# speechLabBcCuny/onssen

Hardware: AMD Instinct MI355X
Metric: real_time_factor (higher is better)
Workload: dtype f32 as split-bf16 (bf16x3 MFMA, fp32 accumulate)

## Files before the change

### include/onssen_hip.h

```cpp
#ifndef ONSSEN_HIP_H
#define ONSSEN_HIP_H

#include <stddef.h>
#include <stdint.h>

#ifdef __cplusplus
extern "C" {
#endif

#define ONSSEN_ABI_VERSION 14

#define ONSSEN_OK 0
#define ONSSEN_E_ARG (-1)
#define ONSSEN_E_WORKSPACE (-2)
#define ONSSEN_E_ALIGN (-3)
#define ONSSEN_WAV_TRUNCATED 1
#define ONSSEN_WAV_E_OPEN (-16)
#define ONSSEN_WAV_E_FORMAT (-17)
#define ONSSEN_WAV_E_UNSUPPORTED (-18)
#define ONSSEN_WAV_E_SOME_FAILED (-19)

#define ONSSEN_BLSTM_SPLIT_ROWS 1
#define ONSSEN_BLSTM_BF16X3 2
#define ONSSEN_BLSTM_XCD 4
// ... 73 lines not shown
                           int group, float eps, float* C, int R, int64_t c_s0, int64_t c_s1, float* C2, int64_t c2_s0,
                           int64_t c2_s1, int bf16_only, void* stream);
int onssen_linear_x3p_norms(const uint16_t* a_img, int M, int K, const uint16_t* w_img, const float* bias, int N, int group,
                            float eps, float* C, float* inv_norm, void* stream);

int onssen_linear_x3p_resid(const uint16_t* a_img, int M, int K, const uint16_t* w_img, const float* bias, int N, int group,
                            float eps, const float* resid, int resid_mod, float* C, int R, int64_t c_s0, int64_t c_s1,
                            int bf16_only, void* stream);

#define ONSSEN_BLSTM_WS_HEADER_BYTES 32768
size_t onssen_blstm_workspace_bytes(int B, int T, int in_dim, int H, int L, int ug);
int onssen_blstm_y_image(int B, int T, int in_dim, int H, int L, int ug, size_t* offset_bytes, int* KB);
int onssen_blstm_x_image(int B, int T, int in_dim, int H, int L, int ug, size_t* offset_bytes, int* KB);
int onssen_blstm_forward_f32(const float* x, int64_t xs_b, int64_t xs_t, int B, int T, int in_dim, int H, int L,
                             int ug, const float* const* wih_p_host, const float* const* whh_p_host,
                             const float* const* bias_p_host, float* y, void* ws, size_t ws_bytes, int flags,
                             void* stream);

size_t onssen_blstm_pipe2_workspace_bytes(int B, int T, int in_dim, int H, int ug);
int onssen_blstm_pipe2_y_image(int B, int T, int in_dim, int H, int ug, size_t* offset_bytes, int* KB);
int onssen_blstm_pipe2_forward_f32(const float* x, int64_t xs_b, int64_t xs_t, int B, int T, int in_dim, int H, int ug,
                                   const float* const* wih_p_host, const float* const* whh_p_host,
                                   const float* const* bias_p_host, void* ws, size_t ws_bytes, int flags, void* stream);
int onssen_blstm_pipe2_forward_ragged_f32(const float* x, int64_t xs_b, int64_t xs_t, int B, int T_cap, int T, const int32_t* frames,
                                          int T_prev, const int32_t* frames_prev, int in_dim, int H, int ug,
                                          const float* const* wih_p_host, const float* const* whh_p_host,
                                          const float* const* bias_p_host, void* ws, size_t ws_bytes, int flags, void* stream);

#define ONSSEN_LSTM_BWD_STEPS 0
#define ONSSEN_LSTM_BWD_XCD 1
int onssen_lstm_train_forward_f32(const float* x, int64_t x_stride_b, int64_t x_stride_t, int B, int T, int in_dim, int H,
                                  int ug, const uint16_t* wih_img, const uint16_t* whh_x3, const float* bias_p, float* y,
                                  float* gates, float* cs, void* ws, size_t ws_bytes, void* stream);
int onssen_lstm_train_backward_img_f32(int B, int T, int H, int ug, const uint16_t* whh_img, const float* dy, const float* gates,
                                       const float* cs, void* ws, size_t ws_bytes, float* db_rows, uint16_t* dp_img, void* stream);
int onssen_lstm_train_forward_form_f32(const float* x, int64_t x_stride_b, int64_t x_stride_t, int B, int T, int in_dim, int H,
                                       int ug, const void* wih, const void* whh, const float* bias_p, float* y, float* gates,
                                       float* cs, void* ws, size_t ws_bytes, int flags, void* stream);
int64_t onssen_lstm_whhT_elems(int H, int ug);
int onssen_lstm_pack_whhT_bf16x3(const float* w_hh, int H, int ug, uint16_t* out, void* stream);
int64_t onssen_lstm_whhR_elems(int H, int ug);
int onssen_lstm_pack_whhR_bf16x3(const float* w_hh, int H, int ug, uint16_t* out, void* stream);
size_t onssen_lstm_train_backward_workspace_bytes(int B, int H, int ug, int form);
int onssen_lstm_train_backward_f32(int B, int T, int H, int ug, const uint16_t* whh_img, const float* dy, float* gates_dp,
                                   const float* cs, void* ws, size_t ws_bytes, int form, float* db_rows, void* stream);
int onssen_dropout_f32(const float* x, int64_t n, float p, uint64_t seed, float* out, void* stream);
// ... 215 lines not shown
```

### onssen_amd/_abi.py

```python
import ctypes as C
import os

EPI_BIAS, EPI_L2NORM, EPI_SIGMOID, EPI_RELU = 0, 1, 2, 3
ENHANCE_MSA, ENHANCE_PSA = 0, 1
EPI_BF16 = 0x100
ABI_VERSION = 14
WAV_TRUNCATED = 1
BLSTM_SPLIT_ROWS = 1
BLSTM_BF16X3 = 2
BLSTM_XCD = 4
BLSTM_FUSE_IN0 = 16
BLSTM_FUSE_TAIL = 32
BLSTM_BF16 = 64
BLSTM_G_READY = 128
BLSTM_WS_DIRTY = 65536
LSTM_BWD_STEPS, LSTM_BWD_XCD = 0, 1
DC_CLUSTER_LAUNCH_PER_ITERATION = 1
BLSTM_WS_HEADER = 32768
TASNET_GLN, TASNET_CLN, TASNET_BN = 0, 1, 2
TASNET_RELU, TASNET_SIGMOID, TASNET_SOFTMAX = 0, 1, 2
TASNET_RAGGED_MAX = 64
TASNET_F32, TASNET_BF16X3, TASNET_BF16 = 0, 1, 2

_vp, _i, _i64, _f, _sz = C.c_void_p, C.c_int, C.c_int64, C.c_float, C.c_size_t
# ... 7 lines not shown
    "onssen_lstm_geometry_x3": (_i, [_i, _i, C.POINTER(_i), C.POINTER(_i), C.POINTER(_i64)]),
    "onssen_lstm_pack_whh_bf16x3": (_i, [_vp, _i, _i, _vp, _vp]),
    "onssen_lstm_pack_wih_bf16x3": (_i, [_vp, _i, _i, _i, _vp, _vp]),
    "onssen_lstm_pack_f32": (_i, [_vp, _vp, _vp, _vp, _i, _i, _i, _i, _vp, _vp, _vp, _vp]),
    "onssen_lstm_pack_train_f32": (_i, [_i, _i, _i, _i, _vp, _vp, _vp, _vp, _vp, _vp, _vp, _vp, _vp, _vp]),
    "onssen_lstm_pack_wih_image_f32": (_i, [_vp, _vp, _vp, _i, _i, _i, _i, _vp, _vp, _vp, _vp]),
    "onssen_clip_adam_workspace_bytes": (_sz, [_vp, _i]),
    "onssen_clip_adam_f32": (_i, [_i, _vp, _vp, _vp, _vp, _vp, _f, C.c_double, C.c_double, C.c_double, C.c_double, _i, _i, _vp, _sz, _vp]),
    "onssen_head_pack_f32": (_i, [_vp, _vp, _i, _i, _i, _vp, _vp, _vp, _vp, _f, _vp, _vp, _vp]),
    "onssen_linear_f32": (_i, [_vp, _i64, _i64, _i, _i, _i, _vp, _i, _vp, _i, _i, _i, _f, _vp, _vp, _i64, _i64, _vp]),
    "onssen_linear_pack_bf16x3": (_i, [_vp, _i, _i, _i, _i, _vp, _vp]),
    "onssen_linear_bf16x3": (_i, [_vp, _i64, _i64, _i, _i, _i, _vp, _i, _vp, _i, _i, _i, _f, _vp, _vp, _i64, _i64, _vp]),
    "onssen_x3_image_f32": (_i, [_vp, _i64, _i64, _i, _i, _i, _vp, _vp]),
    "onssen_linear_x3p": (_i, [_vp, _i, _i, _vp, _vp, _i, _i, _i, _f, _vp, _i, _i64, _i64, _vp]),
    "onssen_linear_x3p_resid": (_i, [_vp, _i, _i, _vp, _vp, _i, _i, _f, _vp, _i, _vp, _i, _i64, _i64, _i, _vp]),
    "onssen_linear_x3p_pair": (_i, [_vp, _i, _i, _vp, _vp, _i, _i, _i, _f, _vp, _i, _i64, _i64, _vp, _i64, _i64, _i, _vp]),
    "onssen_blstm_workspace_bytes": (_sz, [_i, _i, _i, _i, _i, _i]),
    "onssen_blstm_y_image": (_i, [_i, _i, _i, _i, _i, _i, _vp, _vp]),
    "onssen_blstm_x_image": (_i, [_i, _i, _i, _i, _i, _i, _vp, _vp]),
    "onssen_blstm_forward_f32": (_i, [_vp, _i64, _i64, _i, _i, _i, _i, _i, _i, _pp, _pp, _pp, _vp, _vp, _sz, _i, _vp]),
    "onssen_blstm_pipe2_workspace_bytes": (_sz, [_i, _i, _i, _i, _i]),
    "onssen_blstm_pipe2_y_image": (_i, [_i, _i, _i, _i, _i, _vp, _vp]),
    "onssen_blstm_pipe2_forward_f32": (_i, [_vp, _i64, _i64, _i, _i, _i, _i, _i, _pp, _pp, _pp, _vp, _sz, _i, _vp]),
    "onssen_blstm_pipe2_forward_ragged_f32": (_i, [_vp, _i64, _i64, _i, _i, _i, _vp, _i, _vp, _i, _i, _i, _pp, _pp, _pp, _vp, _sz, _i, _vp]),
    "onssen_linear_x3p_batched": (_i, [_vp, _i64, _i, _i, _vp, _i64, _vp, _i, _vp, _i64, _i64, _i, _vp]),
    "onssen_linear_x3p_batched_split": (_i, [_vp, _i64, _i, _i, _vp, _i64, _vp, _i, _i, _vp, _i64, _i64, _i64, _i, _vp, _i64, _i64, _i64,
                                             _i, _vp]),
    "onssen_linear_x3p_batched_split_alt": (_i, [_vp, _i64, _i, _i, _vp, _i64, _vp, _i, _i, _vp, _i64, _i64, _i64, _i, _vp, _i64, _i64,
                                                 _i64, _i, _i, _vp]),
    "onssen_linear_x3t": (_i, [_vp, _vp, _i, _i, _i, _vp, _vp, _i64, _vp]),
    "onssen_lstm_wgrad_images_f32": (_i, [_vp, _vp, _vp, _i, _i, _i, _i, _i, _vp, _i, _vp, _i64, _i64, _i64, _vp, _i64, _i64, _i64, _vp]),
    "onssen_x3_image_t_f32": (_i, [_vp, _i64, _i, _i, _i, _vp, _vp]),
    "onssen_x3_image_both_f32": (_i, [_vp, _i64, _i, _i, _vp, _vp, _vp]),
    "onssen_x3_image_both_colsum_f32": (_i, [_vp, _i64, _i, _i, _vp, _vp, _vp, _vp]),
    "onssen_lstm_train_forward_f32": (_i, [_vp, _i64, _i64, _i, _i, _i, _i, _i, _vp, _vp, _vp, _vp, _vp, _vp, _vp, _sz, _vp]),
    "onssen_lstm_train_forward_form_f32": (_i, [_vp, _i64, _i64, _i, _i, _i, _i, _i, _vp, _vp, _vp, _vp, _vp, _vp, _vp, _sz, _i, _vp]),
    "onssen_lstm_whhT_elems": (_i64, [_i, _i]),
    "onssen_lstm_pack_whhT_bf16x3": (_i, [_vp, _i, _i, _vp, _vp]),
    "onssen_lstm_whhR_elems": (_i64, [_i, _i]),
    "onssen_lstm_pack_whhR_bf16x3": (_i, [_vp, _i, _i, _vp, _vp]),
    "onssen_lstm_train_backward_workspace_bytes": (_sz, [_i, _i, _i, _i]),
    "onssen_lstm_train_backward_f32": (_i, [_i, _i, _i, _i, _vp, _vp, _vp, _vp, _vp, _sz, _i, _vp, _vp]),
    "onssen_lstm_train_backward_img_f32": (_i, [_i, _i, _i, _i, _vp, _vp, _vp, _vp, _vp, _sz, _vp, _vp, _vp]),
    "onssen_dropout_f32": (_i, [_vp, _i64, _f, C.c_uint64, _vp, _vp]),
    "onssen_l2norm_rows_f32": (_i, [_vp, _i64, _i, _f, _vp, _vp]),
    "onssen_bn_rows_workspace_bytes": (_sz, [_i64, _i]),
# ... 382 lines not shown
        if frames is not None:
            self.check(self.dll.onssen_blstm_forward_ragged_f32(x, xs_b, xs_t, B, T, frames, in_dim, H, L, ug, arr(*wih_ptrs),
                                                                arr(*whh_ptrs), arr(*bias_ptrs), y, ws, ws_bytes, flags, stream),
                       "onssen_blstm_forward_ragged_f32")
            return
        self.check(self.dll.onssen_blstm_forward_f32(x, xs_b, xs_t, B, T, in_dim, H, L, ug, arr(*wih_ptrs),
                                                     arr(*whh_ptrs), arr(*bias_ptrs), y, ws, ws_bytes, flags, stream),
                   "onssen_blstm_forward_f32")

    def blstm_pipe2_workspace_bytes(self, B, T, in_dim, H, ug):
        return int(self.dll.onssen_blstm_pipe2_workspace_bytes(B, T, in_dim, H, ug))

    def blstm_pipe2_y_image(self, B, T, in_dim, H, ug):
        off, kb = C.c_size_t(0), C.c_int(0)
        self.check(self.dll.onssen_blstm_pipe2_y_image(B, T, in_dim, H, ug, C.byref(off), C.byref(kb)), "onssen_blstm_pipe2_y_image")
        return int(off.value), int(kb.value)

    def blstm_pipe2_forward(self, x, xs_b, xs_t, B, T, in_dim, H, ug, wih_ptrs, whh_ptrs, bias_ptrs, ws, ws_bytes, flags, stream):
        arr = C.c_void_p * 2
        self.check(self.dll.onssen_blstm_pipe2_forward_f32(x, xs_b, xs_t, B, T, in_dim, H, ug, arr(*wih_ptrs), arr(*whh_ptrs),
                                                           arr(*bias_ptrs), ws, ws_bytes, flags, stream),
                   "onssen_blstm_pipe2_forward_f32")

    def blstm_pipe2_forward_ragged(self, x, xs_b, xs_t, B, T_cap, T, frames, T_prev, frames_prev, in_dim, H, ug, wih_ptrs, whh_ptrs,
                                   bias_ptrs, ws, ws_bytes, flags, stream):
        arr = C.c_void_p * 2
        self.check(self.dll.onssen_blstm_pipe2_forward_ragged_f32(x, xs_b, xs_t, B, T_cap, T, frames, T_prev, frames_prev, in_dim, H, ug,
                                                                  arr(*wih_ptrs), arr(*whh_ptrs), arr(*bias_ptrs), ws, ws_bytes, flags,
                                                                  stream),
                   "onssen_blstm_pipe2_forward_ragged_f32")

    def linear_x3p_batched(self, a_img, a_bs, M, K, w_img, w_bs, bias, N, out, c_bs, ldc, batch, stream):
        self.check(self.dll.onssen_linear_x3p_batched(a_img, a_bs, M, K, w_img, w_bs, bias, N, out, c_bs, ldc, batch, stream),
                   "onssen_linear_x3p_batched")

    def linear_x3p_batched_split(self, a_img, a_bs, M, K, w_img, w_bs, bias, N, R, out, c_bs, c_s0, c_s1, n_split, out2, c2_bs,
                                 c2_s0, c2_s1, batch, stream):
        self.check(self.dll.onssen_linear_x3p_batched_split(a_img, a_bs, M, K, w_img, w_bs, bias, N, R, out, c_bs, c_s0, c_s1, n_split,
                                                            out2, c2_bs, c2_s0, c2_s1, batch, stream), "onssen_linear_x3p_batched_split")

    def linear_x3p_batched_split_alt(self, a_img, a_bs, M, K, w_img, w_bs, bias, N, R, out, c_bs, c_s0, c_s1, n_split, out2, c2_bs,
                                     c2_s0, c2_s1, n_split_odd, batch, stream):
        self.check(self.dll.onssen_linear_x3p_batched_split_alt(a_img, a_bs, M, K, w_img, w_bs, bias, N, R, out, c_bs, c_s0, c_s1,
                                                                n_split, out2, c2_bs, c2_s0, c2_s1, n_split_odd, batch, stream),
                   "onssen_linear_x3p_batched_split_alt")

# ... 213 lines not shown
```

### onssen_amd/csrc/labels_cluster.inc

```
__global__ void utt_max_kernel(const float* __restrict__ x, long per_utt, float* __restrict__ out) {
  __shared__ float red[256];
  const float* p = x + (long)blockIdx.x * per_utt;
  float m = -INFINITY;
  for (long i = threadIdx.x; i < per_utt; i += 256) m = fmaxf(m, p[i]);
  red[threadIdx.x] = m;
  __syncthreads();
  for (int s = 128; s > 0; s >>= 1) {
    if ((int)threadIdx.x < s) red[threadIdx.x] = fmaxf(red[threadIdx.x], red[threadIdx.x + s]);
    __syncthreads();
  }
  if (threadIdx.x == 0) out[blockIdx.x] = red[0];
}

__global__ void labels_kernel(const float* __restrict__ mix, const float* __restrict__ s1, const float* __restrict__ s2,
                              const float* __restrict__ feat, const float* __restrict__ fmax, long per_utt, long total,
                              float db_threshold, float* __restrict__ one_hot, float* __restrict__ mag_mix,
                              float* __restrict__ mag_s1, float* __restrict__ mag_s2, float* __restrict__ cos_s1,
                              float* __restrict__ cos_s2) {
  for (long e = (long)blockIdx.x * blockDim.x + threadIdx.x; e < total; e += (long)gridDim.x * blockDim.x) {
    const float xr = mix[2 * e], xi = mix[2 * e + 1];
    const float ar = s1[2 * e], ai = s1[2 * e + 1], br = s2[2 * e], bi = s2[2 * e + 1];
    const float m1 = hypotf(ar, ai), m2 = hypotf(br, bi);
    mag_mix[e] = hypotf(xr, xi);
    mag_s1[e] = m1;
// ... 760 lines not shown
  for (long t0 = i_lo; t0 < i_hi; t0 += 256) {
    const long i = t0 + tid;
    const int act = (i < i_hi && f[i] >= thr) ? 1 : 0;
    scan[tid] = act;
    __syncthreads();
    for (int off = 1; off < 256; off <<= 1) {
      const int v = tid >= off ? scan[tid - off] : 0;
      __syncthreads();
      scan[tid] += v;
      __syncthreads();
    }
    if (i < i_hi) dst[i] = act ? base + scan[tid] - act : -1;
    const int tot = scan[255];
    __syncthreads();
    base += tot;
  }
  for (long i = nb + (long)blockIdx.x * 256 + tid; i < per_utt; i += (long)NBLK * 256) dst[i] = -1;
  if (blockIdx.x == 0) {
    float* wb = const_cast<float*>(ws) + (long)b * ws_stride;
    for (int k = tid; k < 2 * NBP * (D + 4); k += 256) wb[1 + 2 * D + k] = __builtin_bit_cast(float, 1u);
  }
}

template <int DT>
__global__ __launch_bounds__(256) void kmeans2_mask_compact_kernel(const float* __restrict__ comp, const int* __restrict__ dest,
                                                                   long per_utt, int D_rt, const float* __restrict__ ws,
                                                                   long ws_stride, float* __restrict__ masks) {
  using namespace km;
  constexpr int DC = DT ? DT : DMAX;
  const int D = DT ? DT : D_rt;
  const int b = blockIdx.y, tid = threadIdx.x;
  const float* e = comp + (long)b * per_utt * D;
  const int* dst = dest + (long)b * per_utt;
  const float* w = ws + (long)b * ws_stride;
  float c0[DC], c1[DC];
  float q0 = 0.f, q1 = 0.f;
#pragma unroll
  for (int d = 0; d < DC; ++d) {
    c0[d] = d < D ? w[1 + d] : 0.f; c1[d] = d < D ? w[1 + D + d] : 0.f;
    q0 += c0[d] * c0[d]; q1 += c1[d] * c1[d];
  }
  for (long i = (long)blockIdx.x * 256 + tid; i < per_utt; i += (long)gridDim.x * 256) {
    const int row = dst[i];
    int lab = 0;
    if (row >= 0) {
      float v[DC];
// ... 24 lines not shown
```

### onssen_amd/csrc/lstm.inc

```
struct StepArgs {
  const float* G = nullptr;
  const float* whh = nullptr;
  float* y = nullptr;
  float* c = nullptr;
  const unsigned short* whh_x3 = nullptr;
  unsigned short* hs = nullptr;
  int KQ2 = 0, Hs = 0;
  int B = 0, T = 0, Hp = 0, NP = 0, KQ = 0, NU = 0, step = 0;
  long long* dbg = nullptr;
  int ablate = 0;
  const int* frames = nullptr;
  float* save_g = nullptr;
  float* save_c = nullptr;
};

namespace rec {
constexpr int RLD = 72;
constexpr int QB = 10;
constexpr int QB3 = 5;
}

__device__ __forceinline__ float gate_sigmoid(float x) {
  return __builtin_amdgcn_rcpf(1.0f + __builtin_amdgcn_exp2f(-1.4426950408889634f * x));
}
// ... 296 lines not shown
  const unsigned short* ximg = nullptr;
  const float* bias0 = nullptr;
  int KC0 = 0;
  int KCM = 0;
  const float* x0 = nullptr;
  long xs_b = 0, xs_t = 0;
  const float* wtail = nullptr;
  float* save_g = nullptr;
  float* save_c = nullptr;
  int terms = 0;
  int RG = 0;
  unsigned spin_limit = 0;
  long long* dbg = nullptr;
  int ablate = 0;
  unsigned short* yimg = nullptr;
  int KBI = 0;
  const int* frames = nullptr;
  int nbg_a = 0;
  const float* G_b = nullptr;
  const unsigned short* whh_b = nullptr;
  unsigned short* yimg_b = nullptr;
  int T_b = 0;
  const int* frames_b = nullptr;
};

template <int J>
__device__ __forceinline__ unsigned quad_bcast(unsigned v) {
  return (unsigned)__builtin_amdgcn_update_dpp(0, (int)v, J * 0x55, 0xf, 0xf, false);
}

template <int NT, int NW, bool FUSE, int TERMS, bool STACK, bool SAVE = false, bool RAGGED = false>
__global__ __launch_bounds__(64 * NW) void lstm_xcd_kernel(XcdArgs p) {
  static_assert(!STACK || TERMS == 3, "stacking is a property of the split form");
  constexpr bool F32 = TERMS == 0;
  static_assert(!F32 || (!FUSE && !SAVE), "the exact-fp32 form is the plain inference recurrence");
  static_assert(NW == 8, "waves 5..7 never own elements: they stage the input projection");
  static_assert(!RAGGED || (TERMS == 3 && STACK && !FUSE && !SAVE), "ragged batches: the plain stacked split-bf16 inference recurrence");
  constexpr int UG = 4 * NT;
  constexpr int NE = 16 * UG;
  constexpr int NTHR = 64 * NW;
  constexpr int EPT = (NE + NTHR - 1) / NTHR;
  constexpr bool PAIRED = ONSSEN_XCD_PAIRED && STACK && !FUSE && NT >= 2;
  constexpr int NTA = PAIRED ? (NT + 1) / 2 : NT;
  constexpr int NKP = PAIRED ? 4 : NW;
  constexpr int CPW = F32 ? 40 / NW + (40 % NW != 0) : PAIRED ? 5 : 20 / NW + (20 % NW != 0);
  constexpr int CHB = F32 ? 1024 : 2048;
  constexpr int NHL = TERMS == 3 ? 2 : 1;
  constexpr int NLD = (TERMS == 3 && !STACK) ? 2 : 1;
  constexpr int PBS = 320, PTS = 4 * PBS + 16;
  constexpr unsigned TAG = F32 ? 0x40000000u : 0x4000u;
  constexpr int NGRP = tile_group_count(ONSSEN_XCD_TILE_GROUPS);
  constexpr bool GROUPED = !F32 && !PAIRED && NGRP > 1 && tile_group_sum(ONSSEN_XCD_TILE_GROUPS) == NT;
  __shared__ __attribute__((aligned(16))) char part_s[2 * NKP * NT * PTS];
  __shared__ __attribute__((aligned(16))) u32x4 share_s[PAIRED ? 4 * CPW * NLD * 64 : 1];
  __shared__ unsigned share_flag[4];
  constexpr int KCMAX = 4;
  __shared__ unsigned s_ctl[3];
  __shared__ unsigned s_done[8];
#ifndef ONSSEN_XCD_PROFILE_STN
#define ONSSEN_XCD_PROFILE_STN 64
#endif
  constexpr int ST0 = 64, STN = ONSSEN_XCD_PROFILE_STN;
  constexpr bool PROF = ONSSEN_XCD_PROFILE != 0;
  constexpr int ABL = ONSSEN_XCD_ABLATE;
  constexpr int DELAY_CELL = ONSSEN_XCD_DELAY_CELL ? ONSSEN_XCD_DELAY_CELL : (!STACK && TERMS == 3 && !FUSE) ? ONSSEN_XCD_DELAY_CELL_U
                             : (STACK && !SAVE) ? ONSSEN_XCD_DELAY_CELL_S : SAVE ? ONSSEN_XCD_DELAY_CELL_T : 0;
  constexpr int CELL_PRIO = ONSSEN_XCD_CELL_PRIO ? ONSSEN_XCD_CELL_PRIO : (!STACK && TERMS == 3 && !FUSE) ? ONSSEN_XCD_CELL_PRIO_U : 0;
  __shared__ long long stamp_s[PROF ? STN * 24 : 1];
  const int tid = threadIdx.x, lane = tid & 63;
  const int wave = __builtin_amdgcn_readfirstlane(tid >> 6);
  const int ugi = blockIdx.x >> 3, g = (p.ablate & 8) ? ((blockIdx.x + ugi) & 7) : (blockIdx.x & 7);
  if (PROF && p.dbg && tid == 0)
    p.dbg[4096 + blockIdx.x] = (long long)(__builtin_amdgcn_s_getreg(6164) & 15u) |
                               ((long long)__builtin_amdgcn_s_getreg(63492) << 8);
  if (g >= 2 * p.nbg) return;
  const int dir = g / p.nbg;
  int bg = g % p.nbg;
  if (p.nbg_a > 0 && bg >= p.nbg_a) {
    bg -= p.nbg_a;
    p.G = p.G_b; p.whh = p.whh_b; p.yimg = p.yimg_b; p.y = nullptr;
    if constexpr (RAGGED) { p.T = p.T_b; p.frames = p.frames_b; }
  }
  const int RG = p.RG;
  const int b0 = p.row0 + bg * RG;
  unsigned* abort_w = p.sync + 280;
  const long hx_group = (long)g * 2 * p.KQ2 * 1024;
  const int KQX = F32 ? (p.Hp + 15) / 16 : p.KQ2;

  const int qj = tid & 3;
  const unsigned lo_delta = STACK ? (unsigned)RG * 16u : 1024u;
  const long g_step = (long)p.B * 2 * p.NP, y_step = (long)p.B * 2 * p.Hp, i_step = (long)p.B * p.KBI * 64;
  bool e_ok[EPT], e_inb[EPT];
  unsigned g_off[EPT], y_off[EPT];
// ... 657 lines not shown
```

### onssen_amd/csrc/lstm_run.inc

```

struct LstmGeo {
  int ug, Hp, NP, NU;
  int KQ;
  int KQ2, Hs;
  int KQB, NUB;
};
static bool lstm_geo(int H, int ug, LstmGeo* g) {
  if (H <= 0 || ug < 4 || ug > 24 || (ug % 4) != 0) return false;
  g->ug = ug; g->Hp = ceil_div(H, ug) * ug; g->NP = 4 * g->Hp; g->NU = g->Hp / ug;
  g->KQ = ceil_div(g->Hp, 16); g->KQ2 = ceil_div(g->Hp, 32); g->Hs = 32 * g->KQ2;
  g->KQB = ceil_div(g->NP, 32); g->NUB = ceil_div(g->Hp, 16);
  return true;
}
int onssen_lstm_geometry(int H, int ug, int* Hp, int* NP, int* KQ, int64_t* whh_elems) {
  LstmGeo g;
  if (!lstm_geo(H, ug, &g)) return ONSSEN_E_ARG;
  if (Hp) *Hp = g.Hp;
  if (NP) *NP = g.NP;
  if (KQ) *KQ = g.KQ;
  if (whh_elems) *whh_elems = (int64_t)g.NU * g.KQ * (ug / 4) * 256;
  return ONSSEN_OK;
}
int onssen_lstm_geometry_x3(int H, int ug, int* KQ2, int* Hs, int64_t* whh_x3_elems) {
  LstmGeo g;
// ... 135 lines not shown
    } else if constexpr (NT < 6) {
      if (xa.terms == 0) {
        ONSSEN_XCD_LAUNCH(false, 0, false, false, false);
      } else if (xa.terms == 1) {
        if (fz) ONSSEN_XCD_LAUNCH(true, 1, false, false, false); else ONSSEN_XCD_LAUNCH(false, 1, false, false, false);
      } else {
        if (stack) ONSSEN_XCD_LAUNCH(true, 3, true, false, false); else ONSSEN_XCD_LAUNCH(true, 3, false, false, false);
      }
    }
  }
#undef ONSSEN_XCD_LAUNCH
  hipError_t e = hipGetLastError();
  return e == hipSuccess ? ONSSEN_OK : (int)e;
}

template <int NT>
static int launch_xcd_pair(XcdArgs xa, hipStream_t st) {
  if (xa.B > 32 || xa.terms != 3 || xa.KC0 > 0 || xa.save_c || !xa.G_b || !xa.whh_b || !xa.yimg_b) return ONSSEN_E_ARG;
  if ((xa.frames != nullptr) != (xa.frames_b != nullptr) || (xa.frames && xa.B > 16)) return ONSSEN_E_ARG;
  xa.RG = xa.B <= 16 ? 8 : 16;
  xa.row0 = 0;
  xa.nbg_a = ceil_div(xa.B, xa.RG);
  xa.nbg = 2 * xa.nbg_a;
  const dim3 grid((unsigned)(8 * xa.NU));
  if (xa.frames) hipLaunchKernelGGL((lstm_xcd_kernel<NT, 8, false, 3, true, false, true>), grid, dim3(512), 0, st, xa);
  else if (xa.RG == 8) hipLaunchKernelGGL((lstm_xcd_kernel<NT, 8, false, 3, true, false>), grid, dim3(512), 0, st, xa);
  else hipLaunchKernelGGL((lstm_xcd_kernel<NT, 8, false, 3, false, false>), grid, dim3(512), 0, st, xa);
  hipError_t e = hipGetLastError();
  return e == hipSuccess ? ONSSEN_OK : (int)e;
}

struct BlstmRun {
  const float* x; int64_t xs_b, xs_t; int B, T, in_dim, L, flags;
  const float* const* wih; const float* const* whh; const float* const* bias;
  float *y, *save_g, *save_c; const int32_t* frames; void* stream;
  LstmGeo g; BlstmWs o; char* ws;
  float *G, *ybuf; uint16_t *img_x, *img_ab[2]; long long* dbg;
  bool x3, xcd;
  bool images;
  bool bf16_only;
  bool fuse0(int l) const { return images && l == 0 && (flags & ONSSEN_BLSTM_FUSE_IN0); }
  float* yout(int l) const { return (L - 1 - l) % 2 == 0 ? y : ybuf; }
  const float* yin(int l) const { return (L - 1 - l) % 2 == 0 ? ybuf : y; }
};

static int blstm_plan(BlstmRun& r, int H, int ug, void* ws, size_t ws_bytes) {
  const int flags = r.flags;
  if (!lstm_geo(H, ug, &r.g)) return ONSSEN_E_ARG;
// ... 155 lines not shown
  return blstm_forward_impl(x, xs_b, xs_t, B, T, in_dim, H, L, ug, wih_p_host, whh_p_host, bias_p_host, y, ws, ws_bytes,
                            flags, stream, nullptr, nullptr, frames);
}

int onssen_lstm_train_forward_f32(const float* x, int64_t xs_b, int64_t xs_t, int B, int T, int in_dim, int H, int ug,
                                  const uint16_t* wih_img, const uint16_t* whh_x3, const float* bias_p, float* y,
                                  float* gates, float* cs, void* ws, size_t ws_bytes, void* stream) {
  return onssen_lstm_train_forward_form_f32(x, xs_b, xs_t, B, T, in_dim, H, ug, wih_img, whh_x3, bias_p, y, gates, cs, ws, ws_bytes,
                                            ONSSEN_BLSTM_BF16X3 | ONSSEN_BLSTM_XCD, stream);
}

int onssen_lstm_train_forward_form_f32(const float* x, int64_t xs_b, int64_t xs_t, int B, int T, int in_dim, int H, int ug,
                                       const void* wih, const void* whh, const float* bias_p, float* y, float* gates,
                                       float* cs, void* ws, size_t ws_bytes, int flags, void* stream) {
  if (!y || !gates || !cs || !aligned16(gates)) return ONSSEN_E_ARG;
  const int form = flags & (ONSSEN_BLSTM_XCD | ONSSEN_BLSTM_BF16X3);
  if ((flags & ~(ONSSEN_BLSTM_XCD | ONSSEN_BLSTM_BF16X3)) != 0 || form == ONSSEN_BLSTM_XCD) return ONSSEN_E_ARG;
  const float* wih_a[1] = {(const float*)wih};
  const float* whh_a[1] = {(const float*)whh};
  const float* bias[1] = {bias_p};
  return blstm_forward_impl(x, xs_b, xs_t, B, T, in_dim, H, 1, ug, wih_a, whh_a, bias, y, ws, ws_bytes, flags, stream, gates, cs);
}

static int blstm_pipe2_impl(const float* x, int64_t xs_b, int64_t xs_t, int B, int T_cap, int T, const int32_t* frames, int T_prev,
                            const int32_t* frames_prev, int in_dim, int H, int ug, const float* const* wih_p_host,
                            const float* const* whh_p_host, const float* const* bias_p_host, void* ws, size_t ws_bytes, int flags,
                            void* stream) {
  LstmGeo g;
  Pipe2Ws o;
  if (!lstm_geo(H, ug, &g)) return ONSSEN_E_ARG;
  if (!x || !ws || !wih_p_host || !whh_p_host || !bias_p_host || B <= 0 || B > 32 || T <= 0 || in_dim <= 0) return ONSSEN_E_ARG;
  if (T > T_cap || T_prev <= 0 || T_prev > T_cap) return ONSSEN_E_ARG;
  if ((frames != nullptr) != (frames_prev != nullptr) || (frames && B > 16)) return ONSSEN_E_ARG;
  if ((flags & 0xff & ~ONSSEN_BLSTM_G_READY) != (ONSSEN_BLSTM_BF16X3 | ONSSEN_BLSTM_XCD)) return ONSSEN_E_ARG;
  const bool g_ready = (flags & ONSSEN_BLSTM_G_READY) != 0;
  if (!pipe2_ws_layout(B, T_cap, in_dim, g, &o)) return ONSSEN_E_ARG;
  if (ws_bytes < o.total) return ONSSEN_E_WORKSPACE;
  if (!aligned256(ws)) return ONSSEN_E_ALIGN;
  if (ug > 20 || g.NU > 32 || g.KQ2 > 24) return ONSSEN_E_ARG;
  char* base = (char*)ws;
  float *G0 = (float*)(base + o.g0), *G1 = (float*)(base + o.g1);
  uint16_t *img_x = (uint16_t*)(base + o.img_x), *img0 = (uint16_t*)(base + o.img0), *img1 = (uint16_t*)(base + o.img1);
  const int NP = g.NP;
  int rc = ONSSEN_OK;
  if (!g_ready) {
    rc = onssen_x3_image_f32(x, xs_t, xs_b, B, T * B, in_dim, img_x, stream);
    if (rc != ONSSEN_OK) return rc;
    rc = onssen_linear_x3p(img_x, T * B, in_dim, (const uint16_t*)wih_p_host[0], bias_p_host[0], 2 * NP, ONSSEN_EPI_BIAS, 0, 0.f, G0, B,
                           (int64_t)B * 2 * NP, 2 * NP, stream);
    if (rc != ONSSEN_OK) return rc;
  }
  XcdArgs xa = xcd_args(g, ws, o.hs, B, flags);
  xa.G = G1; xa.whh = (const unsigned short*)whh_p_host[1]; xa.yimg = img1; xa.T = T_prev; xa.frames = frames_prev;
  xa.G_b = G0; xa.whh_b = (const unsigned short*)whh_p_host[0]; xa.yimg_b = img0; xa.T_b = T; xa.frames_b = frames;
  xa.ximg = img_x; xa.bias0 = bias_p_host[0]; xa.x0 = x; xa.xs_b = (long)xs_b; xa.xs_t = (long)xs_t;
  xa.terms = 3;
  ONSSEN_CLEAR_ERROR();
  rc = dispatch_ug<20>(ug, [&](auto ugc) { return launch_xcd_pair<decltype(ugc)::value / 4>(xa, (hipStream_t)stream); });
  if (rc != ONSSEN_OK || g_ready) return rc;
  return onssen_linear_x3p(img0, T * B, 2 * g.Hp, (const uint16_t*)wih_p_host[1], bias_p_host[1], 2 * NP, ONSSEN_EPI_BIAS, 0, 0.f, G1, B,
                           (int64_t)B * 2 * NP, 2 * NP, stream);
}

int onssen_blstm_pipe2_forward_f32(const float* x, int64_t xs_b, int64_t xs_t, int B, int T, int in_dim, int H, int ug,
                                   const float* const* wih_p_host, const float* const* whh_p_host,
                                   const float* const* bias_p_host, void* ws, size_t ws_bytes, int flags, void* stream) {
  return blstm_pipe2_impl(x, xs_b, xs_t, B, T, T, nullptr, T, nullptr, in_dim, H, ug, wih_p_host, whh_p_host, bias_p_host, ws, ws_bytes,
                          flags, stream);
}

int onssen_blstm_pipe2_forward_ragged_f32(const float* x, int64_t xs_b, int64_t xs_t, int B, int T_cap, int T, const int32_t* frames,
                                          int T_prev, const int32_t* frames_prev, int in_dim, int H, int ug,
                                          const float* const* wih_p_host, const float* const* whh_p_host,
                                          const float* const* bias_p_host, void* ws, size_t ws_bytes, int flags, void* stream) {
  if (!frames || !frames_prev) return ONSSEN_E_ARG;
  return blstm_pipe2_impl(x, xs_b, xs_t, B, T_cap, T, frames, T_prev, frames_prev, in_dim, H, ug, wih_p_host, whh_p_host, bias_p_host, ws,
                          ws_bytes, flags, stream);
}

static size_t bwd_step_image_bytes(int B, const LstmGeo& g) { return align256((size_t)2 * 2 * ceil_div(B, 16) * g.KQB * 2048); }
static size_t bwd_workspace_bytes(int B, const LstmGeo& g, int form) {
  if (form == ONSSEN_LSTM_BWD_XCD)
    return ONSSEN_BLSTM_WS_HEADER_BYTES + align256((size_t)8 * 2 * g.NU * g.NU * xcd_rows_per_group(B, false) * g.ug * sizeof(float));
  return bwd_step_image_bytes(B, g) + align256((size_t)2 * B * g.Hp * sizeof(float));
}
size_t onssen_lstm_train_backward_workspace_bytes(int B, int H, int ug, int form) {
  LstmGeo g;
  return B > 0 && lstm_geo(H, ug, &g) ? bwd_workspace_bytes(B, g, form) : 0;
}

static int lstm_train_backward_impl(int B, int T, int H, int ug, const uint16_t* whh_img, const float* dy, float* gates_dp,
// ... 80 lines not shown
```

### onssen_amd/separation.py

```python
import numpy as np
import torch

from . import options
from .features import mask_istft, stft_logmag
from .nn._core import _XcdStatus, recovering


def _ragged(wav, lengths, hop_size):
    if lengths is None:
        return None, None
    from .features import _lengths_i32
    lengths = _lengths_i32(lengths, wav.shape[0], wav.shape[-1], wav.device, "lengths", lo=hop_size)
    return lengths, (1 + lengths // hop_size).to(torch.int32)


def _misi_iters(iters, who):
    import numbers
    if isinstance(iters, bool) or not isinstance(iters, numbers.Integral) or iters < 0:
        raise ValueError(f"{who}: the number of MISI iterations must be a non-negative integer, got {iters!r}")
    return int(iters)


@torch.no_grad()
def misi(stft_ri, masks, wav, iters, hop_size=64, frames=None, lengths=None, phases=None):
# ... 397 lines not shown

    def _post(self, parities):
        from .nn._core import _XcdStatus
        _XcdStatus.post(self.ws)
        for q in parities:
            _XcdStatus.post_cluster(self.cws[q], self.cstat)

    @torch.no_grad()
    def flush(self):
        from .nn._core import _XcdStatus
        if self.count == 0:
            return None
        out = self._drain(self.count & 1)
        self.count = 0
        _XcdStatus.flush()
        return out

    def reset(self):
        self.count = 0


class DCPipeline(_DCPipeCore):

    def __init__(self, model, B, n_samples, window_size=256, hop_size=64, db_threshold=40.0, iters=20, tol=1e-4, graph=True):
        from .nn._core import _version_key
        why = _dc_pipe_why_not(model, B, window_size, 32)
        if why:
            raise RuntimeError(f"DCPipeline needs {why}; use separate_dc")
        self.n = int(n_samples)
        self.T = T = 1 + self.n // int(hop_size)
        super().__init__(model, B, T, window_size, hop_size, db_threshold, iters, tol)
        dev, F = self.dev, self.F
        mk = lambda *s: torch.empty(*s, device=dev, dtype=torch.float32)
        self.wav = [torch.zeros(B, self.n, device=dev) for _ in range(2)]
        self.logmag = [mk(B, T, F) for _ in range(2)]
        self.ri = [mk(B, T, F, 2) for _ in range(2)]
        self.out = [torch.zeros(B, 2, self.n, device=dev) for _ in range(2)]
        self.masks = mk(B, T, F, 2)
        self.graphs = [None, None]
        self.use_graph = bool(graph)
        self._wkey = None
        self._version_key = _version_key
        self._prime()

    def _enqueue(self, p, back_end=True):
        lib, B, T, F = self.lib, self.B, self.T, self.F
        st = torch.cuda.current_stream().cuda_stream
        pk = self.model._packed.get(self.ug)
        lib.stft_logmag(self.wav[p].data_ptr(), B, self.n, self.n, self.nfft, self.hop, 1e-7, self.logmag[p].data_ptr(),
                        self.ri[p].data_ptr(), st)
        lib.dc_index(self.logmag[p].data_ptr(), B, T, F, self.D, self.db, self.cws[p].data_ptr(), self.cnb, st)
        lib.blstm_pipe2_forward(self.logmag[p].data_ptr(), T * F, F, B, T, F, self.H, self.ug,
                                [t.data_ptr() for t in pk.wih_img], [t.data_ptr() for t in pk.whh_x3], [t.data_ptr() for t in pk.bias],
                                self.ws.data_ptr(), self.wnb, self.flags, st)
        if back_end:
            m = self.masks
            self._back_end(pk, 1 - p, T, self.comp_off, self.dest_off, self.ri[1 - p], (m.stride(0), m.stride(3), m.stride(1), m.stride(2)),
                           self.n, self.out[p], st)

    def _prime(self):
        from .nn._core import _XcdStatus
        _XcdStatus.poll()
        for p in (0, 1):
            self._enqueue(p, back_end=p == 1)
        self._post((0, 1))
        self.count = 0

    def _capture(self):
        key = self._version_key(self.model.rnn.flat_weights() + [self.model.fc_dc.weight, self.model.bn.running_mean])
        if self._wkey == key and self.graphs[0] is not None:
            return
        pk = self.model._packed.get(self.ug)
        self.model._head.get(pk.Hp)
        torch.cuda.synchronize(self.dev)
        self.graphs = [None, None]
        s = torch.cuda.Stream(self.dev)
        s.wait_stream(torch.cuda.current_stream(self.dev))
# ... 227 lines not shown
```

Baseline: 66140.

## Fuse deep-clustering index map into BLSTM pair launch as auxiliary workgroups

```diff
diff --git a/include/onssen_hip.h b/include/onssen_hip.h
--- a/include/onssen_hip.h
+++ b/include/onssen_hip.h
@@ -119,6 +119,10 @@
 int onssen_blstm_pipe2_forward_f32(const float* x, int64_t xs_b, int64_t xs_t, int B, int T, int in_dim, int H, int ug,
                                    const float* const* wih_p_host, const float* const* whh_p_host,
                                    const float* const* bias_p_host, void* ws, size_t ws_bytes, int flags, void* stream);
+int onssen_blstm_pipe2_map_forward_f32(const float* x, int64_t xs_b, int64_t xs_t, int B, int T, int in_dim, int H, int ug,
+                                       const float* const* wih_p_host, const float* const* whh_p_host,
+                                       const float* const* bias_p_host, void* ws, size_t ws_bytes, int flags, float db_threshold, int D,
+                                       void* map_ws, size_t map_ws_bytes, void* stream);
 int onssen_blstm_pipe2_forward_ragged_f32(const float* x, int64_t xs_b, int64_t xs_t, int B, int T_cap, int T, const int32_t* frames,
                                           int T_prev, const int32_t* frames_prev, int in_dim, int H, int ug,
                                           const float* const* wih_p_host, const float* const* whh_p_host,
diff --git a/onssen_amd/_abi.py b/onssen_amd/_abi.py
--- a/onssen_amd/_abi.py
+++ b/onssen_amd/_abi.py
@@ -53,6 +53,7 @@
     "onssen_blstm_pipe2_workspace_bytes": (_sz, [_i, _i, _i, _i, _i]),
     "onssen_blstm_pipe2_y_image": (_i, [_i, _i, _i, _i, _i, _vp, _vp]),
     "onssen_blstm_pipe2_forward_f32": (_i, [_vp, _i64, _i64, _i, _i, _i, _i, _i, _pp, _pp, _pp, _vp, _sz, _i, _vp]),
+    "onssen_blstm_pipe2_map_forward_f32": (_i, [_vp, _i64, _i64, _i, _i, _i, _i, _i, _pp, _pp, _pp, _vp, _sz, _i, _f, _i, _vp, _sz, _vp]),
     "onssen_blstm_pipe2_forward_ragged_f32": (_i, [_vp, _i64, _i64, _i, _i, _i, _vp, _i, _vp, _i, _i, _i, _pp, _pp, _pp, _vp, _sz, _i, _vp]),
     "onssen_linear_x3p_batched": (_i, [_vp, _i64, _i, _i, _vp, _i64, _vp, _i, _vp, _i64, _i64, _i, _vp]),
     "onssen_linear_x3p_batched_split": (_i, [_vp, _i64, _i, _i, _vp, _i64, _vp, _i, _i, _vp, _i64, _i64, _i64, _i, _vp, _i64, _i64, _i64,
@@ -481,6 +482,13 @@
                                                            arr(*bias_ptrs), ws, ws_bytes, flags, stream),
                    "onssen_blstm_pipe2_forward_f32")
 
+    def blstm_pipe2_map_forward(self, x, xs_b, xs_t, B, T, in_dim, H, ug, wih_ptrs, whh_ptrs, bias_ptrs, ws, ws_bytes, flags, db, D,
+                                map_ws, map_ws_bytes, stream):
+        arr = C.c_void_p * 2
+        self.check(self.dll.onssen_blstm_pipe2_map_forward_f32(x, xs_b, xs_t, B, T, in_dim, H, ug, arr(*wih_ptrs), arr(*whh_ptrs),
+                                                               arr(*bias_ptrs), ws, ws_bytes, flags, db, D, map_ws, map_ws_bytes, stream),
+                   "onssen_blstm_pipe2_map_forward_f32")
+
     def blstm_pipe2_forward_ragged(self, x, xs_b, xs_t, B, T_cap, T, frames, T_prev, frames_prev, in_dim, H, ug, wih_ptrs, whh_ptrs,
                                    bias_ptrs, ws, ws_bytes, flags, stream):
         arr = C.c_void_p * 2
diff --git a/onssen_amd/csrc/labels_cluster.inc b/onssen_amd/csrc/labels_cluster.inc
--- a/onssen_amd/csrc/labels_cluster.inc
+++ b/onssen_amd/csrc/labels_cluster.inc
@@ -806,6 +806,113 @@
   }
 }
 
+template <int NTHR>
+__device__ __forceinline__ void kmeans2_block_argmax(const float* __restrict__ f, long lo, long hi, int none, float* rv, int* ri,
+                                                     float& v, int& ix) {
+  const int tid = threadIdx.x;
+  float best = -INFINITY;
+  int bi = none;
+#pragma unroll 8
+  for (long i = lo + tid; i < hi; i += NTHR)
+    if (f[i] > best) { best = f[i]; bi = (int)i; }
+  rv[tid] = best; ri[tid] = bi;
+  __syncthreads();
+  for (int s = NTHR / 2; s > 0; s >>= 1) {
+    if (tid < s && (rv[tid + s] > rv[tid] || (rv[tid + s] == rv[tid] && ri[tid + s] < ri[tid]))) { rv[tid] = rv[tid + s]; ri[tid] = ri[tid + s]; }
+    __syncthreads();
+  }
+  v = rv[0]; ix = ri[0];
+  __syncthreads();
+}
+
+template <int NTHR>
+__device__ __forceinline__ void kmeans2_map_workgroup(const float* __restrict__ feat, long per_utt, float db, float* __restrict__ ws, long ws_stride,
+                                      int* __restrict__ iw, int* __restrict__ dest, int D, int B, int first, int step, char* lds) {
+  using namespace km;
+  static_assert(NBLK == 64 && IW == 72, "the int words of an utterance: 64 chunk counts, then 8 counters");
+  constexpr int NWV = NTHR / 64, RUN = 8;
+  float* rv = reinterpret_cast<float*>(lds);
+  int* ri = reinterpret_cast<int*>(rv + NTHR);
+  int* wtot = ri + NTHR;
+  int* cs = wtot + 2 * NWV;
+  const int tid = threadIdx.x, lane = tid & 63, wv = tid >> 6;
+  const int nb = (int)per_utt;
+  const int chunk = (nb + NBLK - 1) / NBLK;
+  const int ntag = 2 * NBP * (D + 4);
+  for (int b = first; b < B; b += step) {
+    const float* f = feat + (long)b * per_utt;
+    float* w = ws + (long)b * ws_stride;
+    float* part = w + 1 + 2 * D;
+    int* iwb = iw + (long)b * IW;
+    int* dst = dest + (long)b * per_utt;
+    float vmax;
+    int imax;
+    kmeans2_block_argmax<NTHR>(f, 0, nb, nb, rv, ri, vmax, imax);
+    const float thr = vmax - db / 20.0f;
+    int base = 0, par = 0;
+    for (long t0 = 0; t0 < nb; t0 += (long)NTHR * RUN, par ^= 1) {
+      const long i0 = t0 + (long)tid * RUN;
+      int act[RUN], c = 0;
+#pragma unroll
+      for (int r = 0; r < RUN; ++r) {
+        act[r] = (i0 + r < nb && f[i0 + r] >= thr) ? 1 : 0;
+        c += act[r];
+      }
+      int incl = c;
+#pragma unroll
+      for (int o = 1; o < 64; o <<= 1) {
+        const int v = __builtin_bit_cast(int, __shfl(__builtin_bit_cast(float, incl), (lane - o) & 63));
+        if (lane >= o) incl += v;
+      }
+      if (lane == 63) wtot[par * NWV + wv] = incl;
+      __syncthreads();
+      int pos = base + incl - c;
+#pragma unroll
+      for (int k = 0; k < NWV; ++k) {
+        const int t = wtot[par * NWV + k];
+        if (k < wv) pos += t;
+        base += t;
+      }
+      if (i0 < nb) {
+        unsigned kc = ((unsigned)i0 + (unsigned)chunk - 1u) / (unsigned)chunk;
+        long cstart = (long)kc * chunk;
+#pragma unroll
+        for (int r = 0; r < RUN; ++r) {
+          const long i = i0 + r;
+          if (i < nb) {
+            if (i == cstart) { cs[kc] = pos; ++kc; cstart += chunk; }
+            dst[i] = act[r] ? pos : -1;
+            pos += act[r];
+          }
+        }
+      }
+    }
+    __syncthreads();
+    if (tid < NBLK) {
+      const int c_lo = (long)tid * chunk < nb ? cs[tid] : base;
+      const int c_hi = (tid + 1 < NBLK && (long)(tid + 1) * chunk < nb) ? cs[tid + 1] : base;
+      iwb[tid] = c_hi - c_lo;
+    }
+    if (tid < 8) iwb[64 + tid] = tid == 0 ? base : 0;
+    if (tid == 0) {
+      w[0] = vmax;
+      w[ws_stride - 1] = __builtin_bit_cast(float, imax);
+    }
+    for (int k = tid; k < ntag; k += NTHR) part[k] = __builtin_bit_cast(float, 1u);
+    for (int k = ntag / 2; k < NBLK; ++k) {
+      const long lo = (long)k * chunk, hi = lo + chunk < nb ? lo + chunk : nb;
+      float v;
+      int ix;
+      kmeans2_block_argmax<NTHR>(f, lo, hi, nb, rv, ri, v, ix);
+      if (tid == 0) {
+        part[2 * k] = v;
+        part[2 * k + 1] = __builtin_bit_cast(float, ix);
+      }
+    }
+    __syncthreads();
+  }
+}
+
 template <int DT>
 __global__ __launch_bounds__(256) void kmeans2_mask_compact_kernel(const float* __restrict__ comp, const int* __restrict__ dest,
                                                                    long per_utt, int D_rt, const float* __restrict__ ws,
diff --git a/onssen_amd/csrc/lstm.inc b/onssen_amd/csrc/lstm.inc
--- a/onssen_amd/csrc/lstm.inc
+++ b/onssen_amd/csrc/lstm.inc
@@ -342,6 +342,13 @@
   unsigned short* yimg_b = nullptr;
   int T_b = 0;
   const int* frames_b = nullptr;
+  int aux_n = 0, aux_D = 0;
+  float aux_db = 0.f;
+  const float* aux_feat = nullptr;
+  long aux_per_utt = 0, aux_stride = 0;
+  float* aux_w = nullptr;
+  int* aux_iw = nullptr;
+  int* aux_dest = nullptr;
 };
 
 template <int J>
@@ -349,9 +356,10 @@
   return (unsigned)__builtin_amdgcn_update_dpp(0, (int)v, J * 0x55, 0xf, 0xf, false);
 }
 
-template <int NT, int NW, bool FUSE, int TERMS, bool STACK, bool SAVE = false, bool RAGGED = false>
+template <int NT, int NW, bool FUSE, int TERMS, bool STACK, bool SAVE = false, bool RAGGED = false, bool AUX = false>
 __global__ __launch_bounds__(64 * NW) void lstm_xcd_kernel(XcdArgs p) {
   static_assert(!STACK || TERMS == 3, "stacking is a property of the split form");
+  static_assert(!AUX || (TERMS == 3 && !FUSE && !SAVE && !RAGGED), "aux workgroups ride in the uniform pair launch");
   constexpr bool F32 = TERMS == 0;
   static_assert(!F32 || (!FUSE && !SAVE), "the exact-fp32 form is the plain inference recurrence");
   static_assert(NW == 8, "waves 5..7 never own elements: they stage the input projection");
@@ -389,6 +397,14 @@
   __shared__ long long stamp_s[PROF ? STN * 24 : 1];
   const int tid = threadIdx.x, lane = tid & 63;
   const int wave = __builtin_amdgcn_readfirstlane(tid >> 6);
+  if constexpr (AUX) {
+    static_assert(sizeof(part_s) >= NTHR * 8 + 512, "the map's scratch fits the partial sums' LDS");
+    if ((int)blockIdx.x >= 8 * p.NU) {
+      kmeans2_map_workgroup<NTHR>(p.aux_feat, p.aux_per_utt, p.aux_db, p.aux_w, p.aux_stride, p.aux_iw, p.aux_dest, p.aux_D, p.B,
+                                  (int)blockIdx.x - 8 * p.NU, p.aux_n, part_s);
+      return;
+    }
+  }
   const int ugi = blockIdx.x >> 3, g = (p.ablate & 8) ? ((blockIdx.x + ugi) & 7) : (blockIdx.x & 7);
   if (PROF && p.dbg && tid == 0)
     p.dbg[4096 + blockIdx.x] = (long long)(__builtin_amdgcn_s_getreg(6164) & 15u) |
diff --git a/onssen_amd/csrc/lstm_run.inc b/onssen_amd/csrc/lstm_run.inc
--- a/onssen_amd/csrc/lstm_run.inc
+++ b/onssen_amd/csrc/lstm_run.inc
@@ -181,8 +181,11 @@
   xa.row0 = 0;
   xa.nbg_a = ceil_div(xa.B, xa.RG);
   xa.nbg = 2 * xa.nbg_a;
-  const dim3 grid((unsigned)(8 * xa.NU));
+  if (xa.aux_n < 0 || (xa.aux_n > 0 && xa.frames)) return ONSSEN_E_ARG;
+  const dim3 grid((unsigned)(8 * xa.NU + xa.aux_n));
   if (xa.frames) hipLaunchKernelGGL((lstm_xcd_kernel<NT, 8, false, 3, true, false, true>), grid, dim3(512), 0, st, xa);
+  else if (xa.aux_n > 0 && xa.RG == 8) hipLaunchKernelGGL((lstm_xcd_kernel<NT, 8, false, 3, true, false, false, true>), grid, dim3(512), 0, st, xa);
+  else if (xa.aux_n > 0) hipLaunchKernelGGL((lstm_xcd_kernel<NT, 8, false, 3, false, false, false, true>), grid, dim3(512), 0, st, xa);
   else if (xa.RG == 8) hipLaunchKernelGGL((lstm_xcd_kernel<NT, 8, false, 3, true, false>), grid, dim3(512), 0, st, xa);
   else hipLaunchKernelGGL((lstm_xcd_kernel<NT, 8, false, 3, false, false>), grid, dim3(512), 0, st, xa);
   hipError_t e = hipGetLastError();
@@ -384,10 +387,11 @@
   return blstm_forward_impl(x, xs_b, xs_t, B, T, in_dim, H, 1, ug, wih_a, whh_a, bias, y, ws, ws_bytes, flags, stream, gates, cs);
 }
 
+struct Pipe2Map { float db = 0.f; int D = 0; void* ws = nullptr; size_t ws_bytes = 0; };
 static int blstm_pipe2_impl(const float* x, int64_t xs_b, int64_t xs_t, int B, int T_cap, int T, const int32_t* frames, int T_prev,
                             const int32_t* frames_prev, int in_dim, int H, int ug, const float* const* wih_p_host,
                             const float* const* whh_p_host, const float* const* bias_p_host, void* ws, size_t ws_bytes, int flags,
-                            void* stream) {
+                            void* stream, const Pipe2Map& map = Pipe2Map()) {
   LstmGeo g;
   Pipe2Ws o;
   if (!lstm_geo(H, ug, &g)) return ONSSEN_E_ARG;
@@ -400,6 +404,12 @@
   if (ws_bytes < o.total) return ONSSEN_E_WORKSPACE;
   if (!aligned256(ws)) return ONSSEN_E_ALIGN;
   if (ug > 20 || g.NU > 32 || g.KQ2 > 24) return ONSSEN_E_ARG;
+  const DcWs ml(B, T, in_dim, map.D);
+  if (map.ws) {
+    if (frames || map.D <= 0 || map.D > km::DMAX || xs_t != in_dim || xs_b != (int64_t)T * in_dim) return ONSSEN_E_ARG;
+    if (map.ws_bytes < ml.compact_bytes) return ONSSEN_E_WORKSPACE;
+    if (!aligned256(map.ws)) return ONSSEN_E_ALIGN;
+  }
   char* base = (char*)ws;
   float *G0 = (float*)(base + o.g0), *G1 = (float*)(base + o.g1);
   uint16_t *img_x = (uint16_t*)(base + o.img_x), *img0 = (uint16_t*)(base + o.img0), *img1 = (uint16_t*)(base + o.img1);
@@ -417,6 +427,11 @@
   xa.G_b = G0; xa.whh_b = (const unsigned short*)whh_p_host[0]; xa.yimg_b = img0; xa.T_b = T; xa.frames_b = frames;
   xa.ximg = img_x; xa.bias0 = bias_p_host[0]; xa.x0 = x; xa.xs_b = (long)xs_b; xa.xs_t = (long)xs_t;
   xa.terms = 3;
+  if (map.ws) {
+    xa.aux_n = B < 16 ? B : 16;
+    xa.aux_D = map.D; xa.aux_db = map.db; xa.aux_feat = x; xa.aux_per_utt = (long)T * in_dim; xa.aux_stride = ml.stride;
+    xa.aux_w = (float*)map.ws; xa.aux_iw = ml.at<int>(map.ws, ml.iw); xa.aux_dest = ml.at<int>(map.ws, ml.dest);
+  }
   ONSSEN_CLEAR_ERROR();
   rc = dispatch_ug<20>(ug, [&](auto ugc) { return launch_xcd_pair<decltype(ugc)::value / 4>(xa, (hipStream_t)stream); });
   if (rc != ONSSEN_OK || g_ready) return rc;
@@ -429,6 +444,17 @@
                                    const float* const* bias_p_host, void* ws, size_t ws_bytes, int flags, void* stream) {
   return blstm_pipe2_impl(x, xs_b, xs_t, B, T, T, nullptr, T, nullptr, in_dim, H, ug, wih_p_host, whh_p_host, bias_p_host, ws, ws_bytes,
                           flags, stream);
+}
+
+int onssen_blstm_pipe2_map_forward_f32(const float* x, int64_t xs_b, int64_t xs_t, int B, int T, int in_dim, int H, int ug,
+                                       const float* const* wih_p_host, const float* const* whh_p_host,
+                                       const float* const* bias_p_host, void* ws, size_t ws_bytes, int flags, float db_threshold, int D,
+                                       void* map_ws, size_t map_ws_bytes, void* stream) {
+  if (!map_ws) return ONSSEN_E_ARG;
+  Pipe2Map map;
+  map.db = db_threshold; map.D = D; map.ws = map_ws; map.ws_bytes = map_ws_bytes;
+  return blstm_pipe2_impl(x, xs_b, xs_t, B, T, T, nullptr, T, nullptr, in_dim, H, ug, wih_p_host, whh_p_host, bias_p_host, ws, ws_bytes,
+                          flags, stream, map);
 }
 
 int onssen_blstm_pipe2_forward_ragged_f32(const float* x, int64_t xs_b, int64_t xs_t, int B, int T_cap, int T, const int32_t* frames,
diff --git a/onssen_amd/separation.py b/onssen_amd/separation.py
--- a/onssen_amd/separation.py
+++ b/onssen_amd/separation.py
@@ -443,7 +443,7 @@
 
 class DCPipeline(_DCPipeCore):
 
-    def __init__(self, model, B, n_samples, window_size=256, hop_size=64, db_threshold=40.0, iters=20, tol=1e-4, graph=True):
+    def __init__(self, model, B, n_samples, window_size=256, hop_size=64, db_threshold=40.0, iters=20, tol=1e-4, graph=True, aux_map=True):
         from .nn._core import _version_key
         why = _dc_pipe_why_not(model, B, window_size, 32)
         if why:
@@ -460,6 +460,7 @@
         self.masks = mk(B, T, F, 2)
         self.graphs = [None, None]
         self.use_graph = bool(graph)
+        self.aux_map = bool(aux_map)
         self._wkey = None
         self._version_key = _version_key
         self._prime()
@@ -470,10 +471,14 @@
         pk = self.model._packed.get(self.ug)
         lib.stft_logmag(self.wav[p].data_ptr(), B, self.n, self.n, self.nfft, self.hop, 1e-7, self.logmag[p].data_ptr(),
                         self.ri[p].data_ptr(), st)
-        lib.dc_index(self.logmag[p].data_ptr(), B, T, F, self.D, self.db, self.cws[p].data_ptr(), self.cnb, st)
-        lib.blstm_pipe2_forward(self.logmag[p].data_ptr(), T * F, F, B, T, F, self.H, self.ug,
-                                [t.data_ptr() for t in pk.wih_img], [t.data_ptr() for t in pk.whh_x3], [t.data_ptr() for t in pk.bias],
-                                self.ws.data_ptr(), self.wnb, self.flags, st)
+        weights = [t.data_ptr() for t in pk.wih_img], [t.data_ptr() for t in pk.whh_x3], [t.data_ptr() for t in pk.bias]
+        if self.aux_map:
+            lib.blstm_pipe2_map_forward(self.logmag[p].data_ptr(), T * F, F, B, T, F, self.H, self.ug, *weights, self.ws.data_ptr(), self.wnb,
+                                        self.flags, self.db, self.D, self.cws[p].data_ptr(), self.cnb, st)
+        else:
+            lib.dc_index(self.logmag[p].data_ptr(), B, T, F, self.D, self.db, self.cws[p].data_ptr(), self.cnb, st)
+            lib.blstm_pipe2_forward(self.logmag[p].data_ptr(), T * F, F, B, T, F, self.H, self.ug, *weights, self.ws.data_ptr(), self.wnb,
+                                    self.flags, st)
         if back_end:
             m = self.masks
             self._back_end(pk, 1 - p, T, self.comp_off, self.dest_off, self.ri[1 - p], (m.stride(0), m.stride(3), m.stride(1), m.stride(2)),
```

Result: faster. 67190, median of 6 (+1.6%).
